# Siyou-Li/u2Tokenizer

Hardware: NVIDIA H100
Metric: ct_volumes_per_sec (higher is better)
Workload: dtype bf16

## Files before the change

### u2tokenizer_b200/csrc/dlinear_wgmma.cu

```cuda
#include <cuda_bf16.h>
#include <math.h>
#include <stdio.h>
#include <stdlib.h>

#include "host_util.h"
#include "ptx.cuh"
#include "u2b200.h"

namespace u2 {

constexpr int kDlN = 16;
constexpr int kDlK = 64;
constexpr int kDlBBytes = kDlN * kDlK * 2;
constexpr int kDlThreads = 384;
constexpr int kDlMmaWarp0 = 8;
constexpr int kDlAccLd = 20;

template <int kM>
struct DlCfg {
  static constexpr int kABytes = kM * kDlK * 2;
  static constexpr int kStageBytes = kABytes + kDlBBytes;
#ifndef U2_DL_STAGES128
#define U2_DL_STAGES128 10
#endif
  static constexpr int kStages = (kM == 128) ? U2_DL_STAGES128 : 18;
  static constexpr int kAccBytes = 2 * kM * kDlAccLd * 4;
  static constexpr int kSmem = kStages * kStageBytes + kAccBytes + 1024 + 512;
};

struct DlinArgs {
  int B, N, K;
  int num_tiles, kblocks;
  float* ws;
  int max_slots;
  int* counters;
  const float* ssq_in;
  float inv_norm_dim, eps;
  const __nv_bfloat16* residual;
  long long ldr;
  void* y;
  long long ldy;
  int y_dtype;
  int silu_pair;
  const float* gamma_next;
  __nv_bfloat16* xg;
  long long ldxg;
  float* ssq_out;
  float* ssq_part;
  int* ssq_ticket;
  float* ssq_zero;
  const int* dep_flags;
  int dep_shift;
  int* out_flags;
  unsigned long long* dbg;
};

constexpr int kDlMaxOps = 4;

struct DlinMulti {
  CUtensorMap tw[kDlMaxOps];
  CUtensorMap tx[kDlMaxOps];
  DlinArgs op[kDlMaxOps];
  int n_ops;
  unsigned int* gridbar;
  const int* step_dev;
  unsigned long long* dbg;
  CUtensorMap tnext[2];
  int next_tiles[2], next_kblocks[2], next_units[2];
  int n_next;
  int pre_stages;
  int lookahead_units;
};

#define U2_STAMP(op, i)                                                                  \
  do {                                                                                   \
    if (mp.dbg) {                                                                        \
      unsigned long long t__;                                                            \
      asm volatile("mov.u64 %0, %%globaltimer;" : "=l"(t__));                           \
      mp.dbg[(blockIdx.x * kDlMaxOps + (op)) * 8 + (i)] = t__;                           \
    }                                                                                    \
  } while (0)

__device__ __forceinline__ unsigned int ld_acquire_u32(const unsigned int* p) {
  unsigned int v;
  asm volatile("ld.acquire.gpu.global.u32 %0, [%1];" : "=r"(v) : "l"(p) : "memory");
  return v;
}

__device__ __forceinline__ float4 ld_relaxed_f4(const float4* p) {
  float4 v;
  asm volatile("ld.relaxed.gpu.global.v4.f32 {%0, %1, %2, %3}, [%4];"
               : "=f"(v.x), "=f"(v.y), "=f"(v.z), "=f"(v.w)
               : "l"(p)
               : "memory");
  return v;
}

__device__ __forceinline__ void grid_barrier_wait(const unsigned int* bar, unsigned int target) {
  unsigned int v, spins = 0;
  do {
    asm volatile("ld.relaxed.gpu.global.u32 %0, [%1];" : "=r"(v) : "l"(bar) : "memory");
    if (++spins == (1u << 24)) {
      printf("u2 dlinear: grid barrier timed out (CTA %d sees %u of %u arrivals): CTAs of the launch are not co-resident\n",
             (int)blockIdx.x, v, target);
      __trap();
    }
  } while (v < target);
  asm volatile("fence.acq_rel.gpu;" ::: "memory");
}

struct UnitIter {
  int tile, kb, kblocks, tile_step;
  int left;
  __device__ __forceinline__ void next() {
    if (++kb == kblocks) {
      kb = 0;
      tile += tile_step;
    }
    --left;
  }
  __device__ __forceinline__ int seg_len() const {
    const int r = kblocks - kb;
    return r < left ? r : left;
  }
};

__device__ __forceinline__ UnitIter make_iter(int num_tiles, int kblocks, bool tiles) {
  UnitIter it;
  it.kblocks = kblocks;
  if (tiles) {
    const int mine = (num_tiles > (int)blockIdx.x) ? (num_tiles - (int)blockIdx.x + (int)gridDim.x - 1) / (int)gridDim.x : 0;
    it.tile = blockIdx.x;
    it.kb = 0;
    it.tile_step = gridDim.x;
    it.left = mine * kblocks;
  } else {
    const long long units = (long long)num_tiles * kblocks;
    const long long G = units < (long long)gridDim.x ? units : (long long)gridDim.x;
    it.tile_step = 1;
    if ((long long)blockIdx.x >= G) {
      it.tile = 0;
      it.kb = 0;
      it.left = 0;
    } else {
      const long long base = units * blockIdx.x / G;
      const long long end = units * (blockIdx.x + 1) / G;
      it.tile = (int)(base / kblocks);
      it.kb = (int)(base - (long long)it.tile * kblocks);
      it.left = (int)(end - base);
    }
  }
  return it;
}

__device__ __forceinline__ void wait_tile_flag(const int* flags, int t, int step, unsigned char* ready, int tag) {
  if (ready[t] == (unsigned char)tag) return;
  const int t4 = t & ~3;
  for (;;) {
    int4 f;
    asm volatile("ld.relaxed.gpu.global.v4.s32 {%0, %1, %2, %3}, [%4];"
                 : "=r"(f.x), "=r"(f.y), "=r"(f.z), "=r"(f.w)
                 : "l"(flags + t4)
                 : "memory");
    if (f.x >= step) ready[t4] = (unsigned char)tag;
    if (f.y >= step) ready[t4 + 1] = (unsigned char)tag;
    if (f.z >= step) ready[t4 + 2] = (unsigned char)tag;
    if (f.w >= step) ready[t4 + 3] = (unsigned char)tag;
    if (ready[t] == (unsigned char)tag) break;
  }
  asm volatile("fence.acq_rel.gpu;" ::: "memory");
  asm volatile("fence.proxy.async;" ::: "memory");
}

template <int kM>
__global__ void __launch_bounds__(kDlThreads, 1)
dlinear_wgmma_kernel(const __grid_constant__ DlinMulti mp) {
  using Cfg = DlCfg<kM>;
  constexpr int kStages = Cfg::kStages;
  constexpr int kABytes = Cfg::kABytes;
  constexpr int kStageBytes = Cfg::kStageBytes;
  constexpr bool kTiles = (kM == 64);
  extern __shared__ uint8_t smem_raw[];
  uint8_t* smem = reinterpret_cast<uint8_t*>((reinterpret_cast<uintptr_t>(smem_raw) + 1023) & ~static_cast<uintptr_t>(1023));
  uint8_t* smem_a = smem;
  uint8_t* smem_b = smem + kStages * kABytes;
  float* smem_acc = reinterpret_cast<float*>(smem + kStages * kStageBytes);
  uint64_t* bars = reinterpret_cast<uint64_t*>(smem + kStages * kStageBytes + Cfg::kAccBytes);
  uint64_t* full_bar = bars;
  uint64_t* empty_bar = bars + kStages;
  uint64_t* acc_full_bar = bars + 2 * kStages;
  uint64_t* acc_empty_bar = bars + 2 * kStages + 2;
  __shared__ unsigned char s_ready[1024];
  if (threadIdx.x < 256) reinterpret_cast<unsigned int*>(s_ready)[threadIdx.x] = 0u;

  const int warp_idx = threadIdx.x / 32;
  const int lane = threadIdx.x % 32;
  const int n_ops = mp.n_ops;

  if (warp_idx == 0 && lane == 0) {
    for (int i = 0; i < n_ops; ++i) {
      tma_prefetch_desc(&mp.tw[i]);
      tma_prefetch_desc(&mp.tx[i]);
    }
  }
  if (warp_idx == 1 && lane == 0) {
    for (int s = 0; s < kStages; ++s) {
      mbar_init(&full_bar[s], 1);
      mbar_init(&empty_bar[s], 4);
    }
    for (int s = 0; s < 2; ++s) {
      mbar_init(&acc_full_bar[s], 4);
      mbar_init(&acc_empty_bar[s], 4);
    }
    fence_barrier_init();
  }
  __syncthreads();
  asm volatile("griddepcontrol.launch_dependents;" ::: "memory");

  if (warp_idx == 0) {
    if (lane == 0) {
      const uint64_t pol_w = l2_policy_evict_first();
      int stage = 0;
      uint32_t phase = 0;
      unsigned int target = 0;
      int step = 0;
      for (int oi = 0; oi < n_ops; ++oi) {
        const DlinArgs& p = mp.op[oi];
        UnitIter it = make_iter(p.num_tiles, p.kblocks, kTiles);
        const int pre_cap = (oi == 0 || mp.pre_stages <= 0 || mp.pre_stages > kStages) ? kStages : mp.pre_stages;
        const int npre = it.left < pre_cap ? it.left : pre_cap;
        int st = stage;
        uint32_t ph = phase;
        UnitIter pre = it;
        for (int j = 0; j < npre; ++j) {
          mbar_wait(&empty_bar[st], ph ^ 1);
          mbar_arrive_expect_tx(&full_bar[st], kStageBytes);
          tma_load_4d_hint(smem_a + st * kABytes, &mp.tw[oi], &full_bar[st], pre.kb * kDlK, pre.tile * kM, 0, 0, pol_w);
          pre.next();
          if (++st == kStages) {
            st = 0;
            ph ^= 1;
          }
        }
        {
          UnitIter la = pre;
          for (int j = 0; j < mp.lookahead_units && la.left > 0; ++j) {
            tma_prefetch_l2_4d(&mp.tw[oi], la.kb * kDlK, la.tile * kM, 0, 0);
            la.next();
          }
        }
        U2_STAMP(oi, 0);
        if (oi == 0) {
          asm volatile("griddepcontrol.wait;" ::: "memory");
          step = *reinterpret_cast<const volatile int*>(mp.step_dev);
          target = (unsigned int)step * gridDim.x;
        } else if (!p.dep_flags) {
          grid_barrier_wait(mp.gridbar + (oi - 1), target);
          asm volatile("fence.proxy.async;" ::: "memory");
        }
        U2_STAMP(oi, 1);
        for (int j = 0; j < npre; ++j) {
          if (oi > 0 && p.dep_flags) wait_tile_flag(p.dep_flags, it.kb >> p.dep_shift, step, s_ready, oi);
          tma_load_4d(smem_b + stage * kDlBBytes, &mp.tx[oi], &full_bar[stage], it.kb * kDlK, 0, 0, 0);
          it.next();
          if (++stage == kStages) {
            stage = 0;
            phase ^= 1;
          }
        }
        while (it.left > 0) {
          mbar_wait(&empty_bar[stage], phase ^ 1);
          mbar_arrive_expect_tx(&full_bar[stage], kStageBytes);
          tma_load_4d_hint(smem_a + stage * kABytes, &mp.tw[oi], &full_bar[stage], it.kb * kDlK, it.tile * kM, 0, 0, pol_w);
          if (oi > 0 && p.dep_flags) wait_tile_flag(p.dep_flags, it.kb >> p.dep_shift, step, s_ready, oi);
          tma_load_4d(smem_b + stage * kDlBBytes, &mp.tx[oi], &full_bar[stage], it.kb * kDlK, 0, 0, 0);
          it.next();
          if (++stage == kStages) {
            stage = 0;
            phase ^= 1;
          }
        }
      }
      for (int jn = 0; jn < mp.n_next; ++jn) {
        UnitIter la = make_iter(mp.next_tiles[jn], mp.next_kblocks[jn], kTiles);
        for (int j = 0; j < mp.next_units[jn] && la.left > 0; ++j) {
          tma_prefetch_l2_4d(&mp.tnext[jn], la.kb * kDlK, la.tile * kM, 0, 0);
          la.next();
        }
      }
    }
  } else if (warp_idx >= kDlMmaWarp0) {
    const int w = warp_idx - kDlMmaWarp0;
    int stage = 0;
    uint32_t phase = 0;
    int acc = 0;
    uint32_t acc_phase = 0;
    for (int oi = 0; oi < n_ops; ++oi) {
      UnitIter it = make_iter(mp.op[oi].num_tiles, mp.op[oi].kblocks, kTiles);
      bool first_unit = true;
      while (it.left > 0) {
        const int seg = it.seg_len();
        float d[kM / 64][8];
        for (int j = 0; j < seg; ++j) {
          mbar_wait(&full_bar[stage], phase);
          if (first_unit) {
            if (threadIdx.x == kDlMmaWarp0 * 32) U2_STAMP(oi, 2);
            first_unit = false;
          }
          const uint64_t a_desc = gmma_desc_sw128(smem_u32(smem_a + stage * kABytes));
          const uint64_t b_desc = gmma_desc_sw128(smem_u32(smem_b + stage * kDlBBytes));
          wgmma_fence();
#pragma unroll
          for (int k = 0; k < kDlK / 16; ++k) {
#pragma unroll
            for (int mh = 0; mh < kM / 64; ++mh)
              wgmma_m64n16k16_ss(d[mh], a_desc + 512 * mh + 2 * k, b_desc + 2 * k, (j == 0 && k == 0) ? 0u : 1u);
          }
          wgmma_commit();
          wgmma_wait<0>();
          if (lane == 0) mbar_arrive(&empty_bar[stage]);
          it.next();
          if (++stage == kStages) {
            stage = 0;
            phase ^= 1;
          }
        }
        mbar_wait(&acc_empty_bar[acc], acc_phase ^ 1);
        float* dst = smem_acc + acc * (kM * kDlAccLd);
#pragma unroll
        for (int mh = 0; mh < kM / 64; ++mh) {
#pragma unroll
          for (int e = 0; e < 8; ++e) {
            const int r = mh * 64 + w * 16 + (lane >> 2) + 8 * ((e >> 1) & 1);
            dst[r * kDlAccLd + 8 * (e >> 2) + 2 * (lane & 3) + (e & 1)] = d[mh][e];
          }
        }
        __syncwarp();
        if (lane == 0) mbar_arrive(&acc_full_bar[acc]);
        if (it.left == 0 && threadIdx.x == kDlMmaWarp0 * 32) U2_STAMP(oi, 3);
        if (++acc == 2) {
          acc = 0;
          acc_phase ^= 1;
        }
      }
    }
  } else if (warp_idx >= 4) {
    const int q = warp_idx - 4;
    const int et = threadIdx.x - 128;
    const int trow = (kM == 128) ? et : (q * 16 + (lane & 15));
    const bool tvalid = (kM == 128) ? true : (lane < 16);
    asm volatile("griddepcontrol.wait;" ::: "memory");
    const unsigned int target = (unsigned int)(*reinterpret_cast<const volatile int*>(mp.step_dev)) * gridDim.x;
    int acc = 0;
    uint32_t acc_phase = 0;
    for (int oi = 0; oi < n_ops; ++oi) {
      const DlinArgs& p = mp.op[oi];
      UnitIter it = make_iter(p.num_tiles, p.kblocks, kTiles);
      bool prev_done = (oi == 0);
      if (oi > 0 && !p.dep_flags) {
        if (et == 0) grid_barrier_wait(mp.gridbar + (oi - 1), target);
        asm volatile("bar.sync 1, 128;" ::: "memory");
        prev_done = true;
      }
      while (it.left > 0) {
        const int tile = it.tile;
        const int seg_kb = it.seg_len();
        it.left -= seg_kb;
        it.kb += seg_kb;
        if (it.kb == it.kblocks) {
          it.kb = 0;
          it.tile += it.tile_step;
        }

        const int row = tile * kM + trow;
        const bool whole = (seg_kb == p.kblocks);
        int gf = (int)blockIdx.x, n_contrib = 0;
        if (!whole) {
          const long long units = (long long)p.num_tiles * p.kblocks;
          const long long G = units < (long long)gridDim.x ? units : (long long)gridDim.x;
          const long long u0 = (long long)tile * p.kblocks;
          gf = (int)(((u0 + 1) * G + units - 1) / units) - 1;
          n_contrib = (int)(((u0 + p.kblocks) * G + units - 1) / units) - 1 - gf;
        }
        const bool finalizer = (gf == (int)blockIdx.x);
        const int nvec = (p.B + 3) >> 2;
        const bool row_ok = tvalid && row < p.N;
        unsigned short res_raw[16];
        float rs[16];
        float gam = 0.f;
        if (finalizer) {
          if (!prev_done) {
            if (et == 0) grid_barrier_wait(mp.gridbar + (oi - 1), target);
            asm volatile("bar.sync 1, 128;" ::: "memory");
            prev_done = true;
          }
#pragma unroll
          for (int b = 0; b < 16; ++b) {
            res_raw[b] = 0;
            rs[b] = 1.f;
            if (b < p.B) {
              if (p.residual && !p.silu_pair && row_ok)
                res_raw[b] = __ldcg(reinterpret_cast<const unsigned short*>(p.residual) + (long long)b * p.ldr + row);
              if (p.ssq_in) rs[b] = __ldcg(p.ssq_in + b);
            }
          }
          if (p.gamma_next && row_ok) gam = __ldg(p.gamma_next + row);
        }

        mbar_wait(&acc_full_bar[acc], acc_phase);
        if (et == 0 && it.left == 0) U2_STAMP(oi, 4);
        uint32_t v[16];
        {
          const uint32_t src = smem_u32(smem_acc + acc * (kM * kDlAccLd) + trow * kDlAccLd);
#pragma unroll
          for (int c = 0; c < 4; ++c) {
            const uint4 x = lds128(src + 16 * c);
            v[4 * c] = x.x; v[4 * c + 1] = x.y; v[4 * c + 2] = x.z; v[4 * c + 3] = x.w;
          }
        }
        __syncwarp();
        if ((threadIdx.x & 31) == 0) mbar_arrive(&acc_empty_bar[acc]);
        if (++acc == 2) {
          acc = 0;
          acc_phase ^= 1;
        }

        float f[16];
#pragma unroll
        for (int b = 0; b < 16; ++b) f[b] = __uint_as_float(v[b]);
        if (!finalizer) {
          const int slot = (int)blockIdx.x - gf - 1;
          float4* dst = reinterpret_cast<float4*>(p.ws + (((long long)tile * p.max_slots + slot) * kM + trow) * kDlN);
          if (tvalid) {
#pragma unroll
            for (int c = 0; c < 4; ++c)
              if (c < nvec) __stcg(dst + c, make_float4(f[4 * c], f[4 * c + 1], f[4 * c + 2], f[4 * c + 3]));
          }
        } else {
          if (et == 0) U2_STAMP(oi, 6);
          if (n_contrib > 0 && tvalid) {
            const long long slot_stride = (long long)kM * kDlN / 4;
            float4* src0 = reinterpret_cast<float4*>(p.ws + (((long long)tile * p.max_slots) * kM + trow) * kDlN);
            const float4 sent = make_float4(__uint_as_float(0xffffffffu), __uint_as_float(0xffffffffu),
                                            __uint_as_float(0xffffffffu), __uint_as_float(0xffffffffu));
#pragma unroll
            for (int c = 0; c < 4; ++c) {
              if (c >= nvec) break;
              constexpr int kMaxSlots = 8;
              for (int s0 = 0; s0 < n_contrib; s0 += kMaxSlots) {
                float4 t[kMaxSlots];
                bool ok;
                unsigned int spins = 0;
                do {
                  ok = true;
#pragma unroll
                  for (int sl = 0; sl < kMaxSlots; ++sl)
                    if (s0 + sl < n_contrib) t[sl] = ld_relaxed_f4(src0 + (s0 + sl) * slot_stride + c);
#pragma unroll
                  for (int sl = 0; sl < kMaxSlots; ++sl)
                    if (s0 + sl < n_contrib) {
                      ok = ok && (__float_as_uint(t[sl].x) != 0xffffffffu) && (__float_as_uint(t[sl].y) != 0xffffffffu) &&
                           (__float_as_uint(t[sl].z) != 0xffffffffu) && (__float_as_uint(t[sl].w) != 0xffffffffu);
                    }
                } while (!ok && ++spins < (1u << 22));
#pragma unroll
                for (int sl = 0; sl < kMaxSlots; ++sl)
                  if (s0 + sl < n_contrib) {
                    f[4 * c] += t[sl].x; f[4 * c + 1] += t[sl].y; f[4 * c + 2] += t[sl].z; f[4 * c + 3] += t[sl].w;
                    __stcg(src0 + (s0 + sl) * slot_stride + c, sent);
                  }
              }
            }
          }
          if (et == 0) U2_STAMP(oi, 7);
          if (p.ssq_zero && tile == 0 && et < 16) p.ssq_zero[et] = 0.f;
          float sq[16];
#pragma unroll
          for (int b = 0; b < 16; ++b) {
            sq[b] = 0.f;
            if (b < p.B) {
              float val = f[b];
              if (p.ssq_in) val *= rsqrtf(rs[b] * p.inv_norm_dim + p.eps);
              if (p.silu_pair) {
                const float me = __bfloat162float(__float2bfloat16(val));
                const float other = __shfl_down_sync(0xffffffffu, me, 1);
                if (row_ok && (trow & 1) == 0) {
                  const float o = __fdividef(me, 1.f + __expf(-me)) * other;
                  reinterpret_cast<__nv_bfloat16*>(p.y)[(long long)b * p.ldy + (row >> 1)] = __float2bfloat16(o);
                }
              } else if (row_ok) {
                val += __bfloat162float(__ushort_as_bfloat16(res_raw[b]));
                if (p.y_dtype == U2_DT_BF16) {
                  const __nv_bfloat16 o = __float2bfloat16(val);
                  reinterpret_cast<__nv_bfloat16*>(p.y)[(long long)b * p.ldy + row] = o;
                  val = __bfloat162float(o);
                } else {
                  reinterpret_cast<float*>(p.y)[(long long)b * p.ldy + row] = val;
                }
                if (p.gamma_next) p.xg[(long long)b * p.ldxg + row] = __float2bfloat16(val * gam);
                sq[b] = val * val;
              }
            }
          }
          if (p.ssq_out) {
            __shared__ float s_sq[4][16];
            __shared__ int s_last;
#pragma unroll
            for (int b = 0; b < 16; ++b) {
              float s = sq[b];
#pragma unroll
              for (int o = 16; o > 0; o >>= 1) s += __shfl_xor_sync(0xffffffffu, s, o);
              if (lane == 0) s_sq[q][b] = s;
            }
            asm volatile("bar.sync 1, 128;" ::: "memory");
            if (et < 16) {
              __stcg(p.ssq_part + (long long)tile * 16 + et, ((s_sq[0][et] + s_sq[1][et]) + s_sq[2][et]) + s_sq[3][et]);
              __threadfence();
            }
            asm volatile("bar.sync 1, 128;" ::: "memory");
            if (et == 0) s_last = (atomicAdd(p.ssq_ticket, 1) == p.num_tiles - 1);
            asm volatile("bar.sync 1, 128;" ::: "memory");
            if (s_last) {
              __shared__ float s_grp[8][16];
              __threadfence();
              const int col = et & 15, grp = et >> 4;
              float t = 0.f;
              for (int i0 = grp; i0 < p.num_tiles; i0 += 32) {
                float v[4];
#pragma unroll
                for (int u = 0; u < 4; ++u) {
                  const int i = i0 + 8 * u;
                  v[u] = (i < p.num_tiles) ? __ldcg(p.ssq_part + (long long)i * 16 + col) : 0.f;
                }
#pragma unroll
                for (int u = 0; u < 4; ++u) {
                  const int i = i0 + 8 * u;
                  if (i < p.num_tiles) {
                    t += v[u];
                    __stcg(p.ssq_part + (long long)i * 16 + col, __uint_as_float(0xffffffffu));
                  }
                }
              }
              s_grp[grp][col] = t;
              asm volatile("bar.sync 1, 128;" ::: "memory");
              if (et < p.B) {
                float tot = 0.f;
#pragma unroll
                for (int g = 0; g < 8; ++g) tot += s_grp[g][et];
                p.ssq_out[et] += tot;
              }
              if (et == 0) *p.ssq_ticket = 0;
            }
          }
          if (p.out_flags) {
            asm volatile("bar.sync 1, 128;" ::: "memory");
            if (et == 0) {
              const int stepv = (int)(target / gridDim.x);
              asm volatile("st.release.gpu.global.s32 [%0], %1;" ::"l"(p.out_flags + tile), "r"(stepv) : "memory");
            }
          }
        }
      }
      if (et == 0) U2_STAMP(oi, 5);
      if (oi + 1 < n_ops) {
        asm volatile("bar.sync 1, 128;" ::: "memory");
        if (et == 0) asm volatile("red.release.gpu.global.add.u32 [%0], 1;" ::"l"(mp.gridbar + oi) : "memory");
      }
    }
  }
}

__global__ void __launch_bounds__(256)
decode_embed_kernel(const long long* __restrict__ ids, const __nv_bfloat16* __restrict__ table,
                    const float* __restrict__ gamma, __nv_bfloat16* __restrict__ x, __nv_bfloat16* __restrict__ xg,
                    float* __restrict__ ssq, float* __restrict__ ssq_zero, int* __restrict__ step_counter, int E,
                    long long vocab) {
  const int b = blockIdx.x;
  if (b == 0 && threadIdx.x == 0 && step_counter) *step_counter += 1;
  long long id = ids[b];
  if (id < 0) id = 0;
  if (id >= vocab) id = vocab - 1;
  const __nv_bfloat16* src = table + id * E;
  float s = 0.f;
  for (int i = threadIdx.x; i < E; i += blockDim.x) {
    const __nv_bfloat16 v = src[i];
    const float f = __bfloat162float(v);
    x[(long long)b * E + i] = v;
    xg[(long long)b * E + i] = __float2bfloat16(f * gamma[i]);
    s += f * f;
  }
  __shared__ float red[8];
#pragma unroll
  for (int o = 16; o > 0; o >>= 1) s += __shfl_xor_sync(0xffffffffu, s, o);
  if ((threadIdx.x & 31) == 0) red[threadIdx.x >> 5] = s;
  __syncthreads();
  if (threadIdx.x == 0) {
    float t = 0.f;
    for (int w = 0; w < (int)(blockDim.x >> 5); ++w) t += red[w];
    ssq[b] = t;
    if (ssq_zero) ssq_zero[b] = 0.f;
  }
}

}

using namespace u2;

static int fill_op(const void* x, const void* w, void* y, const u2_dlinear_desc* d, DlinArgs* p, CUtensorMap* tw,
                   CUtensorMap* tx, int kM) {
  if (!x || !w || !y || !d || !d->ws || !d->counters) return set_error(U2_ERR_ARG, "dlinear: null pointer");
  if (d->B < 1 || d->B > kDlN) return set_error(U2_ERR_UNSUPPORTED, "dlinear: 1 <= B <= 16 (got %d)", d->B);
  if (d->N <= 0 || d->K <= 0 || (d->K % kDlK)) return set_error(U2_ERR_ARG, "dlinear: K must be a positive multiple of 64");
  if ((d->ldx & 7) || (d->ldw & 7)) return set_error(U2_ERR_ARG, "dlinear: ldx/ldw must be multiples of 8");
  if (d->silu_pair && (d->N & 1)) return set_error(U2_ERR_ARG, "dlinear: silu_pair needs an even N");
  if (d->gamma_next && !d->xg) return set_error(U2_ERR_ARG, "dlinear: gamma_next needs xg");
  p->B = d->B; p->N = d->N; p->K = d->K;
  p->num_tiles = (d->N + kM - 1) / kM;
  p->kblocks = d->K / kDlK;
  p->ws = d->ws; p->counters = d->counters;
  p->max_slots = 1;
  if (kM == 128) {
    const long long units = (long long)p->num_tiles * p->kblocks;
    int g = num_sms();
    if (g <= 0) g = 132;
    long long rmin = units / g;
    if (rmin < 1) rmin = 1;
    const long long cmax = (p->kblocks + rmin - 1) / rmin + 1;
    p->max_slots = (int)cmax;
    if ((long long)p->num_tiles * cmax * kM * kDlN > d->ws_elems)
      return set_error(U2_ERR_ARG, "dlinear: workspace too small (%lld fp32 needed for N=%d K=%d)",
                       (long long)p->num_tiles * cmax * kM * kDlN, d->N, d->K);
  }
  p->ssq_in = d->ssq_in;
  p->inv_norm_dim = 1.0f / (float)d->K;
  p->eps = d->eps;
  p->residual = reinterpret_cast<const __nv_bfloat16*>(d->residual);
  p->ldr = d->ldr;
  p->y = y; p->ldy = d->ldy; p->y_dtype = d->y_dtype;
  p->silu_pair = d->silu_pair;
  p->gamma_next = d->gamma_next;
  p->xg = reinterpret_cast<__nv_bfloat16*>(d->xg);
  p->ldxg = d->ldxg;
  p->ssq_out = d->ssq_out;
  p->ssq_part = nullptr;
  p->ssq_ticket = nullptr;
  if (d->ssq_out) {
    const long long slots = (kM == 128) ? (long long)p->num_tiles * p->max_slots * kM * kDlN : 0;
    if (slots + (long long)p->num_tiles * kDlN > d->ws_elems)
      return set_error(U2_ERR_ARG, "dlinear: workspace too small for the sums of squares (%lld fp32 needed for N=%d K=%d)",
                       slots + (long long)p->num_tiles * kDlN, d->N, d->K);
    p->ssq_part = d->ws + slots;
    p->ssq_ticket = d->counters + (d->N + 63) / 64;
  }
  p->ssq_zero = d->ssq_zero;
  p->dep_flags = d->dep_flags;
  p->dep_shift = d->dep_shift;
  p->out_flags = d->out_flags;
  p->dbg = nullptr;
  int rc = make_tmap_bf16_4d(tw, w, d->K, d->N, 1, 1, d->ldw, 0, 0, kDlK, kM);
  if (rc) return rc;
  return make_tmap_bf16_4d(tx, x, d->K, d->B, 1, 1, d->ldx, 0, 0, kDlK, kDlN);
}

template <int kM>
static int launch_multi_t(DlinMulti& mp, int pdl, cudaStream_t stream) {
  static bool configured = false;
  if (!configured) {
    cudaError_t e = cudaFuncSetAttribute(dlinear_wgmma_kernel<kM>, cudaFuncAttributeMaxDynamicSharedMemorySize, DlCfg<kM>::kSmem);
    if (e != cudaSuccess) return set_error(U2_ERR_CUDA, "dlinear: cudaFuncSetAttribute: %s", cudaGetErrorString(e));
    int per_sm = 0;
    e = cudaOccupancyMaxActiveBlocksPerMultiprocessor(&per_sm, dlinear_wgmma_kernel<kM>, kDlThreads, DlCfg<kM>::kSmem);
    if (e != cudaSuccess || per_sm < 1)
      return set_error(U2_ERR_CUDA, "dlinear: kernel cannot be resident on an SM (%s, %d CTA/SM): set U2_MULTI_OP=0",
                       cudaGetErrorString(e), per_sm);
    configured = true;
  }
  int grid = num_sms();
  if (grid <= 0) return set_error(U2_ERR_CUDA, "dlinear: cannot query SM count");
  if (mp.n_ops == 1) {
    const long long work = (kM == 64) ? mp.op[0].num_tiles : (long long)mp.op[0].num_tiles * mp.op[0].kblocks;
    if (work < grid) grid = (int)work;
  }
  cudaLaunchConfig_t cfg = {};
  cfg.gridDim = dim3((unsigned)grid);
  cfg.blockDim = dim3(kDlThreads);
  cfg.dynamicSmemBytes = DlCfg<kM>::kSmem;
  cfg.stream = stream;
  cudaLaunchAttribute attr[1];
  attr[0].id = cudaLaunchAttributeProgrammaticStreamSerialization;
  attr[0].val.programmaticStreamSerializationAllowed = 1;
  cfg.attrs = attr;
  cfg.numAttrs = pdl ? 1 : 0;
  cudaError_t e = cudaLaunchKernelEx(&cfg, dlinear_wgmma_kernel<kM>, mp);
  if (e != cudaSuccess) return set_error(U2_ERR_CUDA, "dlinear launch: %s", cudaGetErrorString(e));
  return U2_OK;
}

static int launch_multi(DlinMulti& mp, int kM, int pdl, cudaStream_t stream) {
  return kM == 64 ? launch_multi_t<64>(mp, pdl, stream) : launch_multi_t<128>(mp, pdl, stream);
}

static inline int tile_m_of(const u2_dlinear_desc* d) { return d->sched == U2_DLIN_TILES64 ? 64 : 128; }


extern "C" U2_API int64_t u2_dlinear_ws_elems(int32_t N, int32_t K) {
  if (N <= 0 || K <= 0) return 0;
  const long long tiles = (N + 127) / 128, kblocks = (K + kDlK - 1) / kDlK;
  int g = num_sms();
  if (g <= 0) g = 132;
  long long rmin = tiles * kblocks / g;
  if (rmin < 1) rmin = 1;
  const long long cmax = (kblocks + rmin - 1) / rmin + 1;
  return tiles * cmax * 128 * kDlN + (N + 63) / 64 * kDlN;
}

extern "C" U2_API int u2_dlinear_bf16(const void* x, const void* w, void* y, const u2_dlinear_desc* d, void* stream) {
  static DlinMulti mp;
  mp.n_ops = 1;
  if (!d) return set_error(U2_ERR_ARG, "dlinear: null descriptor");
  const int kM = tile_m_of(d);
  int rc = fill_op(x, w, y, d, &mp.op[0], &mp.tw[0], &mp.tx[0], kM);
  if (rc) return rc;
  mp.gridbar = nullptr;
  mp.n_next = 0;
  mp.lookahead_units = 0;
  mp.pre_stages = 0;
  mp.dbg = reinterpret_cast<unsigned long long*>(d->dbg);
  mp.step_dev = d->counters;
  return launch_multi(mp, kM, d->pdl, reinterpret_cast<cudaStream_t>(stream));
}

extern "C" U2_API int u2_dlinear_multi_bf16(const void* const* x, const void* const* w, void* const* y,
                                            const u2_dlinear_desc* descs, int32_t n_ops, uint32_t* gridbar,
                                            const int32_t* step_dev, int32_t pdl, const u2_dlinear_next* next,
                                            void* stream) {
  if (!x || !w || !y || !descs) return set_error(U2_ERR_ARG, "dlinear_multi: null pointer");
  if (n_ops < 1 || n_ops > kDlMaxOps) return set_error(U2_ERR_ARG, "dlinear_multi: 1 <= n_ops <= %d", kDlMaxOps);
  if (n_ops > 1 && (!gridbar || !step_dev)) return set_error(U2_ERR_ARG, "dlinear_multi: gridbar / step_dev required");
  static DlinMulti mp;
  mp.n_ops = n_ops;
  const int kM = tile_m_of(&descs[0]);
  for (int i = 0; i < n_ops; ++i) {
    if (tile_m_of(&descs[i]) != kM) return set_error(U2_ERR_ARG, "dlinear_multi: all ops of a launch must share one schedule");
    int rc = fill_op(x[i], w[i], y[i], &descs[i], &mp.op[i], &mp.tw[i], &mp.tx[i], kM);
    if (rc) return rc;
  }
  mp.gridbar = gridbar;
  mp.lookahead_units = next ? next->lookahead_units : 0;
  mp.pre_stages = next ? next->pre_stages : 0;
  mp.n_next = 0;
  if (next) {
    for (int j = 0; j < 2 && j < next->n; ++j) {
      if (!next->w[j] || next->K[j] % kDlK || next->N[j] <= 0) return set_error(U2_ERR_ARG, "dlinear_multi: bad look-ahead weight");
      int rc = make_tmap_bf16_4d(&mp.tnext[j], next->w[j], next->K[j], next->N[j], 1, 1, next->ldw[j], 0, 0, kDlK, kM);
      if (rc) return rc;
      mp.next_tiles[j] = (next->N[j] + kM - 1) / kM;
      mp.next_kblocks[j] = next->K[j] / kDlK;
      mp.next_units[j] = next->units[j];
      mp.n_next = j + 1;
    }
  }
  mp.dbg = reinterpret_cast<unsigned long long*>(descs[0].dbg);
  mp.step_dev = step_dev ? step_dev : descs[0].counters;
  return launch_multi(mp, kM, pdl, reinterpret_cast<cudaStream_t>(stream));
}

extern "C" U2_API int u2_decode_embed_bf16(const int64_t* ids, const void* table, const float* gamma, void* x,
                                           void* xg, float* ssq, float* ssq_zero, int32_t* step_counter, int32_t B,
                                           int32_t E, int64_t vocab, void* stream) {
  if (!ids || !table || !gamma || !x || !xg || !ssq) return set_error(U2_ERR_ARG, "decode_embed: null pointer");
  if (B < 1 || B > kDlN) return set_error(U2_ERR_UNSUPPORTED, "decode_embed: 1 <= B <= 16");
  decode_embed_kernel<<<B, 256, 0, reinterpret_cast<cudaStream_t>(stream)>>>(
      reinterpret_cast<const long long*>(ids), reinterpret_cast<const __nv_bfloat16*>(table), gamma,
      reinterpret_cast<__nv_bfloat16*>(x), reinterpret_cast<__nv_bfloat16*>(xg), ssq, ssq_zero, step_counter, E, vocab);
  U2_CHECK_LAUNCH("decode_embed");
  return U2_OK;
}
```

Baseline: 1.998.

## Batch ssq ticket atomics per op and decouple stats finalize from grid barrier

The epilogue warps no longer spin on the grid barrier themselves. The producer thread now signals a shared-memory mbarrier once it has passed the barrier, and the epilogue waits on that. The sum-of-squares reduction moves from a per-tile ticket atomic with threadfence to one acq_rel atomic per CTA per op. The last CTA publishes an epoch word that dependent finalizers wait on. The aim is to cut global atomics, fences and redundant grid-barrier polling, at the cost of a more intricate cross-CTA ordering protocol and a reused gridbar slot that could race.

After: 2.015, median of 6. About the same (+0.8%).

```diff
diff --git a/u2tokenizer_b200/csrc/dlinear_wgmma.cu b/u2tokenizer_b200/csrc/dlinear_wgmma.cu
--- a/u2tokenizer_b200/csrc/dlinear_wgmma.cu
+++ b/u2tokenizer_b200/csrc/dlinear_wgmma.cu
@@ -72,14 +72,19 @@
   int lookahead_units;
 };
 
+constexpr int kDlDbgRec = 16;
 #define U2_STAMP(op, i)                                                                  \
   do {                                                                                   \
     if (mp.dbg) {                                                                        \
       unsigned long long t__;                                                            \
       asm volatile("mov.u64 %0, %%globaltimer;" : "=l"(t__));                           \
-      mp.dbg[(blockIdx.x * kDlMaxOps + (op)) * 8 + (i)] = t__;                           \
+      mp.dbg[(blockIdx.x * kDlMaxOps + (op)) * kDlDbgRec + (i)] = t__;                   \
     }                                                                                    \
   } while (0)
+
+__device__ __forceinline__ unsigned int stats_epoch(unsigned int step, int oi) {
+  return step * kDlMaxOps + (unsigned int)oi + 1u;
+}
 
 __device__ __forceinline__ unsigned int ld_acquire_u32(const unsigned int* p) {
   unsigned int v;
@@ -190,6 +195,7 @@
   uint64_t* empty_bar = bars + kStages;
   uint64_t* acc_full_bar = bars + 2 * kStages;
   uint64_t* acc_empty_bar = bars + 2 * kStages + 2;
+  uint64_t* dep_bar = bars + 2 * kStages + 4;
   __shared__ unsigned char s_ready[1024];
   if (threadIdx.x < 256) reinterpret_cast<unsigned int*>(s_ready)[threadIdx.x] = 0u;
 
@@ -212,6 +218,7 @@
       mbar_init(&acc_full_bar[s], 4);
       mbar_init(&acc_empty_bar[s], 4);
     }
+    mbar_init(dep_bar, 1);
     fence_barrier_init();
   }
   __syncthreads();
@@ -257,6 +264,7 @@
         } else if (!p.dep_flags) {
           grid_barrier_wait(mp.gridbar + (oi - 1), target);
           asm volatile("fence.proxy.async;" ::: "memory");
+          mbar_arrive(dep_bar);
         }
         U2_STAMP(oi, 1);
         for (int j = 0; j < npre; ++j) {
@@ -350,18 +358,20 @@
     const int trow = (kM == 128) ? et : (q * 16 + (lane & 15));
     const bool tvalid = (kM == 128) ? true : (lane < 16);
     asm volatile("griddepcontrol.wait;" ::: "memory");
-    const unsigned int target = (unsigned int)(*reinterpret_cast<const volatile int*>(mp.step_dev)) * gridDim.x;
+    const unsigned int step = (unsigned int)(*reinterpret_cast<const volatile int*>(mp.step_dev));
+    const unsigned int target = step * gridDim.x;
+    unsigned int* const stats_word = (n_ops > 1) ? mp.gridbar + (n_ops - 1) : nullptr;
     int acc = 0;
     uint32_t acc_phase = 0;
+    uint32_t dep_count = 0;
     for (int oi = 0; oi < n_ops; ++oi) {
       const DlinArgs& p = mp.op[oi];
       UnitIter it = make_iter(p.num_tiles, p.kblocks, kTiles);
       bool prev_done = (oi == 0);
-      if (oi > 0 && !p.dep_flags) {
-        if (et == 0) grid_barrier_wait(mp.gridbar + (oi - 1), target);
-        asm volatile("bar.sync 1, 128;" ::: "memory");
-        prev_done = true;
-      }
+      const bool prev_stats = oi > 0 && mp.op[oi - 1].ssq_out;
+      const uint32_t dep_parity = dep_count & 1;
+      if (oi > 0 && !p.dep_flags) ++dep_count;
+      int n_ssq = 0;
       while (it.left > 0) {
         const int tile = it.tile;
         const int seg_kb = it.seg_len();
@@ -390,8 +400,15 @@
         float gam = 0.f;
         if (finalizer) {
           if (!prev_done) {
-            if (et == 0) grid_barrier_wait(mp.gridbar + (oi - 1), target);
-            asm volatile("bar.sync 1, 128;" ::: "memory");
+            if (prev_stats || p.dep_flags) {
+              if (et == 0) {
+                if (prev_stats) grid_barrier_wait(stats_word, stats_epoch(step, oi - 1));
+                else grid_barrier_wait(mp.gridbar + (oi - 1), target);
+              }
+              asm volatile("bar.sync 1, 128;" ::: "memory");
+            } else {
+              mbar_wait(dep_bar, dep_parity);
+            }
             prev_done = true;
           }
 #pragma unroll
@@ -504,7 +521,6 @@
           }
           if (p.ssq_out) {
             __shared__ float s_sq[4][16];
-            __shared__ int s_last;
 #pragma unroll
             for (int b = 0; b < 16; ++b) {
               float s = sq[b];
@@ -513,58 +529,72 @@
               if (lane == 0) s_sq[q][b] = s;
             }
             asm volatile("bar.sync 1, 128;" ::: "memory");
-            if (et < 16) {
+            if (et < 16)
               __stcg(p.ssq_part + (long long)tile * 16 + et, ((s_sq[0][et] + s_sq[1][et]) + s_sq[2][et]) + s_sq[3][et]);
-              __threadfence();
-            }
             asm volatile("bar.sync 1, 128;" ::: "memory");
-            if (et == 0) s_last = (atomicAdd(p.ssq_ticket, 1) == p.num_tiles - 1);
-            asm volatile("bar.sync 1, 128;" ::: "memory");
-            if (s_last) {
-              __shared__ float s_grp[8][16];
-              __threadfence();
-              const int col = et & 15, grp = et >> 4;
-              float t = 0.f;
-              for (int i0 = grp; i0 < p.num_tiles; i0 += 32) {
-                float v[4];
-#pragma unroll
-                for (int u = 0; u < 4; ++u) {
-                  const int i = i0 + 8 * u;
-                  v[u] = (i < p.num_tiles) ? __ldcg(p.ssq_part + (long long)i * 16 + col) : 0.f;
-                }
-#pragma unroll
-                for (int u = 0; u < 4; ++u) {
-                  const int i = i0 + 8 * u;
-                  if (i < p.num_tiles) {
-                    t += v[u];
-                    __stcg(p.ssq_part + (long long)i * 16 + col, __uint_as_float(0xffffffffu));
-                  }
-                }
-              }
-              s_grp[grp][col] = t;
-              asm volatile("bar.sync 1, 128;" ::: "memory");
-              if (et < p.B) {
-                float tot = 0.f;
-#pragma unroll
-                for (int g = 0; g < 8; ++g) tot += s_grp[g][et];
-                p.ssq_out[et] += tot;
-              }
-              if (et == 0) *p.ssq_ticket = 0;
-            }
+            ++n_ssq;
           }
           if (p.out_flags) {
             asm volatile("bar.sync 1, 128;" ::: "memory");
             if (et == 0) {
-              const int stepv = (int)(target / gridDim.x);
-              asm volatile("st.release.gpu.global.s32 [%0], %1;" ::"l"(p.out_flags + tile), "r"(stepv) : "memory");
+              asm volatile("st.release.gpu.global.s32 [%0], %1;" ::"l"(p.out_flags + tile), "r"((int)step) : "memory");
             }
           }
         }
       }
       if (et == 0) U2_STAMP(oi, 5);
       if (oi + 1 < n_ops) {
+        if (prev_stats && !prev_done && et == 0) grid_barrier_wait(stats_word, stats_epoch(step, oi - 1));
         asm volatile("bar.sync 1, 128;" ::: "memory");
         if (et == 0) asm volatile("red.release.gpu.global.add.u32 [%0], 1;" ::"l"(mp.gridbar + oi) : "memory");
+      }
+      if (n_ssq > 0) {
+        __shared__ int s_last;
+        if (et == 0) {
+          unsigned int old;
+          asm volatile("atom.acq_rel.gpu.global.add.u32 %0, [%1], %2;"
+                       : "=r"(old) : "l"(p.ssq_ticket), "r"((unsigned int)n_ssq) : "memory");
+          s_last = (old + (unsigned int)n_ssq == (unsigned int)p.num_tiles);
+        }
+        asm volatile("bar.sync 1, 128;" ::: "memory");
+        if (s_last) {
+          __shared__ float s_grp[8][16];
+          __threadfence();
+          const int col = et & 15, grp = et >> 4;
+          float t = 0.f;
+          for (int i0 = grp; i0 < p.num_tiles; i0 += 32) {
+            float v[4];
+#pragma unroll
+            for (int u = 0; u < 4; ++u) {
+              const int i = i0 + 8 * u;
+              v[u] = (i < p.num_tiles) ? __ldcg(p.ssq_part + (long long)i * 16 + col) : 0.f;
+            }
+#pragma unroll
+            for (int u = 0; u < 4; ++u) {
+              const int i = i0 + 8 * u;
+              if (i < p.num_tiles) {
+                t += v[u];
+                __stcg(p.ssq_part + (long long)i * 16 + col, __uint_as_float(0xffffffffu));
+              }
+            }
+          }
+          s_grp[grp][col] = t;
+          asm volatile("bar.sync 1, 128;" ::: "memory");
+          if (et < p.B) {
+            float tot = 0.f;
+#pragma unroll
+            for (int g = 0; g < 8; ++g) tot += s_grp[g][et];
+            p.ssq_out[et] += tot;
+          }
+          if (et == 0) *p.ssq_ticket = 0;
+          if (oi + 1 < n_ops) {
+            asm volatile("bar.sync 1, 128;" ::: "memory");
+            if (et == 0) {
+              asm volatile("st.release.gpu.global.u32 [%0], %1;" ::"l"(stats_word), "r"(stats_epoch(step, oi)) : "memory");
+              U2_STAMP(oi, 8);
+            }
+          }
+        }
       }
     }
   }
```
